# dachinzo/ringpop-node

Measured on AMD Instinct MI355X. Metric: ring lookups/s + member-updates merged/s; SWIM round time @100k members, higher is better.
Workload: dtype u32; 1 GPU; C2: 10000-server HashRing x 100 replica points, batched lookupN(n=3) of 36-byte keys, 2^26 keys per step; servers=10000, replica_points=100, total_keys=164550934528, parallelism=keys sharded, ring replicated

## Files before the change

### ringpop-node_amd/csrc/rp_ring.hip

```cpp
#include <algorithm>
#include <chrono>
#include <cstdio>
#include <cstdlib>
#include <cstring>
#include <memory>
#include <mutex>
#include <string>
#include <unordered_map>
#include <vector>

#include "../../include/ringpop_amd.h"
#include "rp_farmhash.h"
#include "rp_philox.h"
#include "rp_hashlong.h"
#include "rp_names.h"
#include "rp_prims.h"

namespace rp {

constexpr uint32_t NIL = 0xFFFFFFFFu;

static bool getenv_flag(const char* name) {
    const char* v = getenv(name);
    return v && *v && *v != '0';
// ... 926 lines not shown
        auto defer = [&](uint32_t kk) {
            const uint32_t sp = atomicAdd(&nslow_tile, 1u);
            if (sp < kSlowPerTile) slow_list[t * kSlowPerTile + sp] = kk;
        };
        constexpr int KH = KPL / LH;
        static_assert(KPL % LH == 0, "whole halves");
#ifdef RP_LK_PROF
        uint64_t t3 = 0;
#endif
#pragma unroll
        for (int hh = 0; hh < LH; hh++) {
        if (hh) __builtin_amdgcn_sched_barrier(0);
        u32x2 rec[KH];
#pragma unroll
        for (int kq = 0; kq < KH; kq++) rec[kq] = lk.index_rec(h[hh * KH + kq]);
        uint32_t lo[KH], bc[KH], ws[KH];
        u32x4 win[KH];
#pragma unroll
        for (int kq = 0; kq < KH; kq++) win[kq] = lk.window(h[hh * KH + kq], rec[kq], lo[kq], bc[kq], ws[kq]);
#ifdef RP_LK_PROF
        if (hh == 0) {
            LK_T(t3h, lo[KH - 1]);
            t3 = t3h;
        }
#endif
#pragma unroll
        for (int kq = 0; kq < KH; kq++) {
            const int k = hh * KH + kq;
            lk.resolve(win[kq], h[k], lo[kq], bc[kq], ws[kq], (uint32_t)(tid + k * kLkThreads), nag, ag[wv], so, cnt_tile,
                       defer);
        }
        }
        LK_T(t4, nag);
        __builtin_amdgcn_fence(__ATOMIC_SEQ_CST, "wavefront");
        for (uint32_t j = lane; j < (nag < AG ? nag : AG); j += 64)
            lk.finish2(lk.load16(ag[wv][0][j]), ag[wv][1][j], ag[wv][2][j], so, cnt_tile, defer);
        LK_T(t5a, nag);
        __syncthreads();
        LK_T(t5, tid);
        if (tid == 0) slow_cnt[t] = nslow_tile;
        u32x4* d4 = reinterpret_cast<u32x4*>(out + base * NEED);
        const u32x4* s4 = reinterpret_cast<const u32x4*>(so);
#pragma unroll
        for (int k = tid; k < TK * NEED / 4; k += kLkThreads) __builtin_nontemporal_store(s4[k], d4 + k);
        __syncthreads();
#ifdef RP_LK_PROF
        LK_T(t6, tid);
        pa[1] += t2 - t0;
        pa[2] += t3 - t2;
        pa[3] += t4 - t3;
        pa[4] += t5a - t4;
        pa[5] += t6 - t5;
        ntl += 1;
        (void)t5;
#endif
    }
#ifdef RP_LK_PROF
    if (lane == 0) {
        for (int i = 0; i < 6; i++) atomicAdd(&g_lk_prof[i], (unsigned long long)pa[i]);
        atomicAdd(&g_lk_prof[6], (unsigned long long)ntl);
    }
#endif
    if constexpr (FUSE) {
        constexpr uint32_t TPP = kLkThreads / kSlowPerTile;
        const uint64_t nt = ntiles > blockIdx.x ? (ntiles - blockIdx.x + gridDim.x - 1) / gridDim.x : 0;
        for (uint64_t i0 = 0; i0 < nt; i0 += TPP) {
            const uint64_t i = i0 + (uint32_t)tid / kSlowPerTile;
            const uint32_t q = (uint32_t)tid % kSlowPerTile;
            if (i < nt) {
                const uint64_t t = blockIdx.x + i * gridDim.x;
                const uint32_t c = slow_cnt[t];
                if (c <= kSlowPerTile) {
                    if (q < c) lookupn_redo(keys, fv, np, (uint32_t)NEED, out, counts, t * TK + slow_list[t * kSlowPerTile + q]);
                } else {
                    for (uint32_t k = q; k < (uint32_t)TK; k += kSlowPerTile) lookupn_redo(keys, fv, np, (uint32_t)NEED, out, counts, t * TK + k);
                }
            }
        }
    }
}

#ifdef RP_LK_PROF
__device__ unsigned long long g_sk_prof[10];
#endif
constexpr int kSortDefault = 256;

template <int THREADS, int NEED>
__global__ __launch_bounds__(THREADS) __attribute__((amdgpu_waves_per_eu(4))) void k_lookupn_sorted(
    const uint8_t* __restrict__ keys, uint64_t ntiles, CompactView cv, uint32_t* __restrict__ out,
    uint8_t* __restrict__ counts, uint32_t* __restrict__ slow_list, uint32_t* __restrict__ slow_cnt) {
    constexpr int LEN = 36, W4 = LEN / 4, KPL = 8, HS = 4;
    constexpr int TK = THREADS * KPL;
    constexpr int NW = THREADS / 64;
    constexpr int SUB = TK / 2048;
    constexpr int SK = TK * W4 / HS, SO = TK * NEED;
    constexpr int BINS = THREADS;
    constexpr int BSH = 32 - (BINS == 256 ? 8 : BINS == 512 ? 9 : 10);
    constexpr int CW = BINS / 2;
    constexpr int WPL = CW / 64;
    static_assert(THREADS == 256 || THREADS == 512 || THREADS == 1024, "whole 2,048-key logical tiles, 13-bit slots, 16-bit bin counters");
    static_assert(2 * TK <= SO && SK <= SO, "the ordered pairs and the key slice fit under the rows");
    __shared__ __attribute__((aligned(16))) uint32_t lds[SO];
    __shared__ uint32_t ag[NW][3][kLkAG];
    __shared__ uint32_t bins[CW];
    __shared__ uint32_t nslow_sub[SUB];
    uint32_t* const sk = lds;
    uint32_t* const so = lds;
    u32x2* const pairs = reinterpret_cast<u32x2*>(lds);
    const int tid = threadIdx.x, lane = tid & 63, wv = tid >> 6;
    const LkStages<NEED, 13> lk(cv);
#ifdef RP_LK_PROF
    uint64_t pa[6] = {0, 0, 0, 0, 0, 0}, ntl = 0;
#endif
    if (tid < CW) bins[tid] = 0;
    if (tid < SUB) nslow_sub[tid] = 0;
    for (uint64_t t = blockIdx.x; t < ntiles; t += gridDim.x) {
        const uint64_t base = t * TK;
        uint32_t h[KPL], kk[KPL];
        LK_T(t0, tid);
        lk_key_stage<64, KPL, HS, true>(keys + (base + (uint64_t)wv * 512) * LEN, sk + wv * (SK / NW), lane, h, [] {}, [] {});
        LK_T(t1, h[KPL - 1]);
        uint32_t rank[KPL];
#pragma unroll
        for (int k = 0; k < KPL; k++) {
            const uint32_t b = h[k] >> BSH, sh = (b & 1u) * 16u;
            rank[k] = (atomicAdd(&bins[b >> 1], 1u << sh) >> sh) & 0xFFFFu;
        }
        __syncthreads();
        if (wv == 0) {
            uint32_t c[WPL], sum = 0;
#pragma unroll
            for (int i = 0; i < WPL; i++) {
                c[i] = bins[lane * WPL + i];
                sum += (c[i] & 0xFFFFu) + (c[i] >> 16);
            }
            uint32_t x = sum;
#pragma unroll
            for (int o = 1; o < 64; o <<= 1) {
                const uint32_t y = __shfl_up(x, o, 64);
                if (lane >= o) x += y;
            }
            uint32_t run = x - sum;
#pragma unroll
            for (int i = 0; i < WPL; i++) {
                const uint32_t a = run, b = run + (c[i] & 0xFFFFu);
                run = b + (c[i] >> 16);
                bins[lane * WPL + i] = a | (b << 16);
            }
        }
        __syncthreads();
#pragma unroll
        for (int k = 0; k < KPL; k++) {
            const uint32_t b = h[k] >> BSH, sh = (b & 1u) * 16u;
            const uint32_t slot = ((bins[b >> 1] >> sh) & 0xFFFFu) + rank[k];
            pairs[slot] = u32x2{h[k], (uint32_t)(wv * 512 + lane + 64 * k)};
        }
        __syncthreads();
#pragma unroll
        for (int k = 0; k < KPL; k++) {
            const u32x2 p = pairs[tid + k * THREADS];
            h[k] = p.x;
            kk[k] = p.y;
        }
        if (tid < CW) bins[tid] = 0;
        if (tid < SUB) nslow_sub[tid] = 0;
        LK_T(t2, kk[KPL - 1]);
        __syncthreads();
        uint32_t nag = 0;
        uint8_t* const cnt_tile = counts ? counts + base : nullptr;
        auto defer = [&](uint32_t k) {
            const uint32_t s = k >> 11;
            const uint32_t sp = atomicAdd(&nslow_sub[s], 1u);
            if (sp < kSlowPerTile) slow_list[(t * SUB + s) * kSlowPerTile + sp] = k & 2047u;
        };
        u32x2 rec[KPL];
#pragma unroll
        for (int k = 0; k < KPL; k++) rec[k] = lk.index_rec(h[k]);
        uint32_t lo[KPL], bc[KPL], ws[KPL];
        u32x4 win[KPL];
#pragma unroll
        for (int k = 0; k < KPL; k++) win[k] = lk.window(h[k], rec[k], lo[k], bc[k], ws[k]);
        LK_T(t3, lo[KPL - 1]);
#pragma unroll
        for (int k = 0; k < KPL; k++) lk.resolve(win[k], h[k], lo[k], bc[k], ws[k], kk[k], nag, ag[wv], so, cnt_tile, defer);
        LK_T(t4, nag);
        __builtin_amdgcn_fence(__ATOMIC_SEQ_CST, "wavefront");
        for (uint32_t j = lane; j < (nag < kLkAG ? nag : kLkAG); j += 64)
            lk.finish2(lk.load16(ag[wv][0][j]), ag[wv][1][j], ag[wv][2][j], so, cnt_tile, defer);
        LK_T(t5a, nag);
        __syncthreads();
        LK_T(t5, tid);
        if (tid < SUB) slow_cnt[t * SUB + tid] = nslow_sub[tid];
        u32x4* d4 = reinterpret_cast<u32x4*>(out + base * NEED);
        const u32x4* s4 = reinterpret_cast<const u32x4*>(so);
#pragma unroll
        for (int k = tid; k < TK * NEED / 4; k += THREADS) __builtin_nontemporal_store(s4[k], d4 + k);
        __syncthreads();
#ifdef RP_LK_PROF
        LK_T(t6, tid);
        pa[0] += t1 - t0;
        pa[1] += t2 - t1;
        pa[2] += t3 - t2;
        pa[3] += t4 - t3;
        pa[4] += t5a - t4;
        pa[5] += t6 - t5;
        ntl += 1;
#endif
    }
#ifdef RP_LK_PROF
    if (lane == 0) {
        for (int i = 0; i < 6; i++) atomicAdd(&g_sk_prof[i], (unsigned long long)pa[i]);
        atomicAdd(&g_sk_prof[6], (unsigned long long)ntl);
    }
#endif
}

constexpr int kWsSlots = 2;
constexpr uint32_t kWsSpin = 1u << 22;
typedef uint32_t u32x3v __attribute__((ext_vector_type(3)));

template <int NP, int NC, int ABL = 0>
__global__ __launch_bounds__((NP + NC) * 64) __attribute__((amdgpu_waves_per_eu(4))) void k_lookupn_ws(const uint8_t* __restrict__ keys, uint64_t nwt,
                                                               CompactView cv, uint32_t* __restrict__ out,
                                                               uint32_t out_bytes, uint8_t* __restrict__ counts,
                                                               uint32_t* __restrict__ slow_list,
                                                               uint32_t* __restrict__ slow_cnt,
                                                               uint32_t* __restrict__ err) {
    constexpr int NEED = 3, KPL = 8, LEN = 36, W4 = LEN / 4;
    constexpr int TK = 64 * KPL;
    constexpr int V4 = TK * W4 / 4;
    constexpr int PER = V4 / 64;
    constexpr uint32_t SPAN = 5 - NEED;
    constexpr uint32_t AG = 64;
    static_assert(V4 % 64 == 0, "wave-tile shape");
    __shared__ __attribute__((aligned(16))) uint32_t stg[NP][V4 * 4];
    __shared__ uint32_t ring[NC][kWsSlots][TK];
    __shared__ uint32_t ag[NC][3][AG];
    __shared__ uint32_t prod[NC], cons[NC], nsl[NC];
    const int tid = threadIdx.x, lane = tid & 63, wv = tid >> 6;
    if (tid < NC) {
        prod[tid] = 0;
        cons[tid] = 0;
    }
    __syncthreads();
    const uint64_t nwg = (nwt + NC - 1) / NC;
    auto wait_ge = [&](uint32_t* p, uint32_t target) {
        for (uint32_t n = 0;; n++) {
            const uint32_t v = __builtin_amdgcn_readfirstlane(__hip_atomic_load(p, __ATOMIC_RELAXED, __HIP_MEMORY_SCOPE_WORKGROUP));
            if (v >= target) break;
            if (n == kWsSpin) {
                if (lane == 0) atomicOr(err, 1u);
                break;
            }
            __builtin_amdgcn_s_sleep(1);
            asm volatile("" ::: "memory");
        }
        asm volatile("" ::: "memory");
    };
    if (wv < NP) {
        const int cnt = (NC - wv + NP - 1) / NP;
        auto item_wt = [&](uint32_t j) -> uint64_t {
            const uint64_t T = blockIdx.x + (uint64_t)(j / cnt) * gridDim.x;
            const uint64_t wt = T * NC + wv + (j % cnt) * NP;
            return T < nwg && wt < nwt ? wt : ~0ull;
        };
        u32x4 pre[PER];
        auto issue = [&](uint64_t wt) {
            const u32x4* s4 = reinterpret_cast<const u32x4*>(keys + wt * (uint64_t)(TK * LEN));
#pragma unroll
            for (int q = 0; q < PER; q++) pre[q] = __builtin_nontemporal_load(s4 + lane + 64 * q);
        };
        uint64_t wt = item_wt(0);
        if (ABL != 1 && wt != ~0ull) issue(wt);
        for (uint32_t j = 0; wt != ~0ull; j++) {
            const uint64_t wn = item_wt(j + 1);
            uint32_t h[KPL];
            if constexpr (ABL == 1) {
#pragma unroll
                for (int k = 0; k < KPL; k++) h[k] = (uint32_t)(wt * TK + lane + 64 * k) * 0x9E3779B1u;
            } else {
                u32x4* st4 = reinterpret_cast<u32x4*>(stg[wv]);
#pragma unroll
                for (int q = 0; q < PER; q++) st4[lane + 64 * q] = pre[q];
                __builtin_amdgcn_wave_barrier();
                if (wn != ~0ull) issue(wn);
#pragma unroll
                for (int k = 0; k < KPL; k++) {
                    uint32_t w[W4];
#pragma unroll
                    for (int x = 0; x < W4; x++) w[x] = stg[wv][(lane + 64 * k) * W4 + x];
                    h[k] = fh::hash32_words<LEN>(w);
                }
            }
            __builtin_amdgcn_wave_barrier();
            const int c = wv + (int)(j % cnt) * NP;
            const uint32_t i = j / cnt;
            wait_ge(&cons[c], i + 1 > (uint32_t)kWsSlots ? i + 1 - kWsSlots : 0u);
// ... 1036 lines not shown
        const uint32_t p = pos[i];
        for (uint32_t q = lane; q < L; q += 64) buf[p + q] = names[b + q];
        if (lane == 0) buf[p + L] = ';';
    }
}

__global__ void k_hash_batch(const uint8_t* __restrict__ bytes, const uint64_t* __restrict__ off, uint64_t n,
                             uint32_t* __restrict__ out) {
    const uint64_t gstride = (uint64_t)gridDim.x * blockDim.x;
    for (uint64_t k = (uint64_t)blockIdx.x * blockDim.x + threadIdx.x; k < n; k += gstride)
        out[k] = fh::hash32(fh::PtrSrc{bytes + off[k]}, (uint32_t)(off[k + 1] - off[k]));
}

__global__ void k_gen_uuid(uint32_t seed, uint64_t k0, uint64_t n, uint32_t* __restrict__ out) {
    const uint64_t gstride = (uint64_t)gridDim.x * blockDim.x;
    for (uint64_t k = (uint64_t)blockIdx.x * blockDim.x + threadIdx.x; k < n; k += gstride) {
        uint32_t w[9];
        uuid_key_words(seed, k0 + k, w);
#pragma unroll
        for (int j = 0; j < 9; j++) out[k * 9 + j] = w[j];
    }
}

}


struct LoadScratch {
    DevBuf<uint32_t> rows;
    DevBuf<unsigned long long> out;
    StreamOrder order;
    void use_on(hipStream_t st) { order.use_on(st); }
};

struct RangeScratch {
    DevBuf<uint32_t> val, mi, mj;
    DevBuf<uint32_t> tot;
    DevBuf<uint8_t> flg;
    DevBuf<uint32_t> io;
    StreamOrder order;
    void use_on(hipStream_t st) { order.use_on(st); }
};

struct HandoffScratch {
    DevBuf<uint32_t> key, dst, src, perm;
    DevBuf<uint8_t> slot;
    DevBuf<uint32_t> rank;
    DevBuf<uint32_t> io;
    StreamOrder order;
    void use_on(hipStream_t st) { order.use_on(st); }
};

struct RouteScratch {
    DevBuf<unsigned long long> plane;
    DevBuf<unsigned long long> meta;
    DevBuf<uint8_t> tr;
    DevBuf<unsigned long long> scan;
    DevBuf<uint8_t> io8;
    DevBuf<uint32_t> io32;
    DevBuf<unsigned long long> io64;
    StreamOrder order;
    void use_on(hipStream_t st) { order.use_on(st); }
};

struct LookupKnobs {
    bool wide;
    bool layout_packed;
    bool nowindow;
    bool ablate_set;
    int ablate;
    bool wpred;
    bool hint;
    bool lds;
    uint64_t lds_grid;
    bool lds_stg;
    int lds_abl;
    bool ws;
    int ws_np, ws_nc;
    uint64_t ws_grid;
    int ws_abl;
    bool kpl_set;
    int kpl;
    int sort_t;
    uint64_t grid;
    bool lean_set;
    bool lean;
    bool half_set;
    int half;
    bool fusefix;
    bool stg_set;
    int stg;
    bool lh_set;
    uint64_t lh;
    uint64_t stghs;
    bool debug;
    bool prof_print;
};
static LookupKnobs lookup_knobs() {
    const auto num = [](const char* v) { return v ? atoi(v) : 0; };
    const auto is0 = [](const char* v) { return v && !strcmp(v, "0"); };
    const char *lay = getenv("RP_RING_LAYOUT"), *abl = getenv("RP_LOOKUP_ABLATE"), *lds = getenv("RP_LOOKUP_LDS"),
               *ws = getenv("RP_LOOKUP_WS"), *kpl = getenv("RP_LOOKUP_KPL"), *sort = getenv("RP_LOOKUP_SORT"),
               *lean = getenv("RP_LOOKUP_LEAN"), *half = getenv("RP_LOOKUP_HALF"), *stg = getenv("RP_LOOKUP_STG");
    LookupKnobs k;
    k.wide = getenv_flag("RP_RING_WIDE");
    k.layout_packed = lay && !strcmp(lay, "packed");
    k.nowindow = getenv_flag("RP_RING_NOWINDOW");
    k.ablate_set = abl != nullptr;
    k.ablate = num(abl);
    k.wpred = !is0(getenv("RP_LOOKUP_WPRED"));
    k.hint = !is0(getenv("RP_LOOKUP_HINT"));
    k.lds = lds ? !strcmp(lds, "1") : kLdsDefault;
    k.lds_grid = env_pos("RP_LOOKUP_LDS_GRID", 0);
    k.lds_stg = (int)env_pos("RP_LOOKUP_LDS_STG", 0) == 1;
    k.lds_abl = num(getenv("RP_LOOKUP_LDS_ABL"));
    k.ws = ws && !is0(ws);
    k.ws_np = 1, k.ws_nc = 3;
    if (k.ws && strchr(ws, ':') && sscanf(ws, "%d:%d", &k.ws_np, &k.ws_nc) != 2) k.ws_np = 0;
    k.ws_grid = env_pos("RP_LOOKUP_WS_GRID", 0);
    k.ws_abl = num(getenv("RP_LOOKUP_WS_ABL"));
    k.kpl_set = kpl != nullptr;
    k.kpl = num(kpl);
    k.sort_t = sort ? atoi(sort) : kSortDefault;
    k.grid = env_pos("RP_LOOKUP_GRID", 0);
    k.lean_set = lean != nullptr;
    k.lean = !is0(lean);
    k.half_set = half != nullptr;
    k.half = num(half);
    k.fusefix = getenv_flag("RP_LOOKUP_FUSEFIX");
    k.stg_set = stg != nullptr;
    k.stg = num(stg);
    k.lh_set = getenv("RP_LOOKUP_LH") != nullptr;
    k.lh = env_pos("RP_LOOKUP_LH", 0);
    k.stghs = env_pos("RP_LOOKUP_STGHS", 8);
    k.debug = getenv_flag("RP_LOOKUP_DEBUG");
    k.prof_print = getenv_flag("RP_LK_PROF_PRINT");
    return k;
}

struct Ring {
    int device = 0;
    hipStream_t st = nullptr;
    uint32_t R = 100;
    NameTable nt;
    std::vector<uint8_t> in_ring;
    std::vector<uint64_t> stamp;
    uint64_t next_stamp = 1;
    uint32_t server_count = 0;
    bool has_checksum = false;
    uint32_t checksum = 0;
    DevBuf<uint32_t> tok, own, tok2, own2, bstart;
    uint32_t M = 0;
    uint32_t bbits = 8;
    DevBuf<uint32_t> ent, pbstart;
    DevBuf<uint32_t> slow, nslow;
    bool packed = false;
    uint32_t pbits = 16;
    DevBuf<uint8_t> cent;
    DevBuf<uint32_t> cidx;
    DevBuf<uint32_t> cidxh;
    bool chint = false;
    bool chint_pending = false;
    bool compact = false;
    uint32_t ccb = 0, cob = 0, cfsh = 0;
    DevBuf<uint8_t> lent;
    DevBuf<uint4> lidx;
    bool lds = false, lds_pending = false;
    uint32_t lng = 0, llg = 0, lfb = 0;
    DevBuf<uint8_t> d_inring;
    DevBuf<uint8_t> ck_buf;
    DevBuf<uint32_t> ck_out;
    DevBuf<uint32_t> ntok, nown, flag, pos, ids_dev, tmpk;
    DevBuf<uint64_t> tmp64;
    DevBuf<uint32_t> scalar;
    DevBuf<uint32_t> io_a, io_b;
    DevBuf<uint8_t> io_keys, io_cnt;
    uint32_t* pin_out = nullptr;
    uint8_t* pin_cnt = nullptr;
    uint32_t* pin_out_dev = nullptr;
    uint8_t* pin_cnt_dev = nullptr;
    DevBuf<uint64_t> io_off;
    SvcLines* svc = nullptr;
    SvcLines* svc_dev = nullptr;
    hipStream_t svc_st = nullptr;
    uint32_t svc_idle_ms = 0, svc_seq = 0;
    std::atomic<bool> svc_live{false};
    std::recursive_mutex svc_mu;
    bool svc_v2 = true;
    DevBuf<uint4> svc_dt;
    uint32_t svc_dtb = 0;
    bool svc_dt_valid = false;
    uint64_t svc_prof[9] = {0, 0, 0, 0, 0, 0, 0, 0, 0};
    DevBuf<uint32_t> grp_own, grp_key, grp_first, grp_dk, grp_dv, grp_rank;
    Scratch ws;
    LoadScratch load_ws;
    RangeScratch range_ws;
    HandoffScratch handoff_ws;
    RouteScratch route_ws;
    uint32_t inring_n = 0;

    RingView view() const {
        return RingView{tok.p, own.p, bstart.p, M, 32u - bbits};
    }
    PackedView pview() const { return PackedView{ent.p, pbstart.p, M, pbits}; }
    CompactView cview(const LookupKnobs& k) const {
        return CompactView{cent.p, cidx.p, M, ccb, cob, cfsh, cfsh == 0, (uint32_t)k.ablate,
                           (uint32_t)(3ull * ((uint64_t)M + kEnt3Pad + 6) + 16), (uint32_t)(8ull << (ccb - 3)),
                           k.wpred ? 1u : 0u, chint && k.hint ? cidxh.p : nullptr};
    }
};

struct Replicas {
    int np;
    uint32_t W;
};
static Replicas replicas(int32_t nrep, uint32_t servers) {
    return {(int)std::min<int64_t>(nrep, servers), nrep > 1 ? (uint32_t)nrep : 1u};
}

static uint32_t ring_intern(Ring& r, const char* s, uint32_t n) {
    const uint32_t id = r.nt.intern(s, n);
    if (id >= r.in_ring.size()) {
        r.in_ring.resize(id + 1, 0);
        r.stamp.resize(id + 1, 0);
    }
    return id;
}

static uint32_t choose_bbits(uint32_t M) {
    uint32_t b = 8;
    while (b < 22 && (1ull << (b + 2)) < M) b++;
    return b;
}

static void ring_build_compact(Ring& r) {
    r.compact = false;
    if (r.M < 64) return;
    uint32_t ob = 1;
// ... 301 lines not shown
        hipLaunchKernelGGL(kern, dim3(g), dim3(kLdsThreads), 0, b.st, b.keys, nwt, lv, b.out, b.counts, r.slow.p,
                           r.nslow.p);
    };
    if (b.need == 3 && k.lds_abl) {
        switch (k.lds_abl) {
            case 1: tiles(k_lookupn_lds<KPL, 3, 0, 1>); break;
            case 2: tiles(k_lookupn_lds<KPL, 3, 0, 2>); break;
            case 3: tiles(k_lookupn_lds<KPL, 3, 0, 3>); break;
            case 4: tiles(k_lookupn_lds<KPL, 3, 0, 4>); break;
            default: tiles(k_lookupn_lds<KPL, 3, 0, 7>); break;
        }
    } else {
        with_need(b.need, [&](auto need) {
            constexpr int N = decltype(need)::value;
            if (k.lds_stg)
                tiles(k_lookupn_lds<KPL, N, 1, 0>);
            else
                tiles(k_lookupn_lds<KPL, N, 0, 0>);
        });
    }
    RP_HIP(hipGetLastError());
    lookupn_tiles_end(r, k, b, nwt, TK, nwt * TK, true, 0,
                      [&](auto done, auto tot, auto over, const uint32_t*) {
                          fprintf(stderr, "[rp] lds lookupN: %llu keys, %llu deferred, %llu overflowed tiles (ng %u fb %u ob %u)\n",
                                  done, tot, over, r.lng, r.lfb, r.cob);
                      });
    return true;
}

static bool lookupn_ws(Ring& r, const LookupKnobs& k, const Batch36& b, const CompactView& cv) {
    const uint64_t n = b.n;
    if (!k.ws || b.need != 3 || k.kpl_set || cv.ablate != 0 || n < 512ull * 4 || n * 12ull >= (1ull << 31))
        return false;
    const int wnp = k.ws_np, wnc = k.ws_nc;
    constexpr uint64_t TK = 512;
    const uint64_t nwt = n / TK;
    r.slow.reserve(nwt * kSlowPerTile + 1);
    r.nslow.reserve(nwt + 2);
    uint32_t* err = r.nslow.p + nwt + 1;
    RP_HIP(hipMemsetAsync(err, 0, 4, b.st));
    const uint64_t nwg = (nwt + (uint64_t)wnc - 1) / (uint64_t)(wnc > 0 ? wnc : 1);
    const uint64_t lds_wg = (uint64_t)wnp * 18432 + (uint64_t)wnc * (kWsSlots * 2048 + 780);
    const uint64_t per_cu = wnp + wnc > 0 ? std::max<uint64_t>(1, std::min<uint64_t>(16 / (uint64_t)(wnp + wnc), 163840 / lds_wg)) : 1;
    const unsigned g = (unsigned)std::min<uint64_t>(nwg, k.ws_grid ? k.ws_grid : (uint64_t)cu_count(r.device) * per_cu);
    using Kernel = decltype(&k_lookupn_ws<1, 3>);
    static const struct { int np, nc, abl; Kernel kern; } shapes[] = {
        {1, 3, 0, k_lookupn_ws<1, 3>},      {2, 6, 0, k_lookupn_ws<2, 6>},      {1, 7, 0, k_lookupn_ws<1, 7>},
        {4, 12, 1, k_lookupn_ws<4, 12, 1>}, {4, 12, 2, k_lookupn_ws<4, 12, 2>}, {4, 12, 0, k_lookupn_ws<4, 12>},
        {2, 2, 0, k_lookupn_ws<2, 2>},      {1, 15, 0, k_lookupn_ws<1, 15>},    {2, 14, 0, k_lookupn_ws<2, 14>}};
    Kernel kern = nullptr;
    for (const auto& s : shapes)
        if (!kern && s.np == wnp && s.nc == wnc && (s.abl == 0 || s.abl == k.ws_abl)) kern = s.kern;
    RP_REQUIRE(kern, "RP_LOOKUP_WS: one of 1:3, 2:6, 1:7, 4:12, 2:2, 1:15, 2:14");
    hipLaunchKernelGGL(kern, dim3(g), dim3((wnp + wnc) * 64), 0, b.st, b.keys, nwt, cv, b.out, (uint32_t)(n * 12ull), b.counts,
                       r.slow.p, r.nslow.p, err);
    RP_HIP(hipGetLastError());
    lookupn_tiles_end(r, k, b, nwt, TK, nwt * TK, true, 2,
                      [&](auto done, auto tot, auto over, const uint32_t* c) {
                          fprintf(stderr, "[rp] ws lookupN %d:%d: %llu keys, %llu deferred, %llu overflowed wave-tiles, err %u\n", wnp,
                                  wnc, done, tot, over, c[nwt + 1]);
                      });
    return true;
}

static void lookupn_compact(Ring& r, const LookupKnobs& k, const Batch36& b, const CompactView& cv) {
    const uint64_t n = b.n;
    const int need = b.need, np = b.np;
    const hipStream_t st = b.st;
    int kpl = k.kpl_set ? k.kpl : (need == 3 ? 8 : 4);
    if (kpl != 1 && kpl != 2 && !((kpl == 3 || kpl == 8) && need == 3)) kpl = 4;
    int sort_t = k.sort_t;
    RP_REQUIRE(sort_t == 0 || sort_t == 256 || sort_t == 512 || sort_t == 1024, "RP_LOOKUP_SORT: one of 0, 256, 512, 1024");
    if (need != 3 || !cv.idxh || cv.ablate != 0 || n < 8ull * (uint64_t)sort_t || k.kpl_set || k.half_set ||
        k.lean_set || k.stg_set || k.lh_set || k.fusefix)
        sort_t = 0;
    const uint64_t stiles = sort_t ? n / (8ull * (uint64_t)sort_t) : 0;
    const uint64_t s0 = stiles * 8ull * (uint64_t)sort_t;
    const uint64_t t0 = s0 / 2048;
    if (!sort_t && n < (uint64_t)kLkThreads * kpl) kpl = 4;
    const uint64_t TK = (uint64_t)kLkThreads * kpl;
    const uint64_t ntiles = (n - s0) / TK, done = s0 + ntiles * TK;
    r.slow.reserve((t0 + ntiles) * kSlowPerTile + 1);
    r.nslow.reserve(t0 + ntiles + 1);
    if (stiles) {
        const unsigned sg = grid_for(stiles, 1, (unsigned)(k.grid ? k.grid : sort_t == 256 ? 4096u : sort_t == 512 ? 8192u : 1024u));
        const auto sorted = [&](auto kern) {
            hipLaunchKernelGGL(kern, dim3(sg), dim3(sort_t), 0, st, b.keys, stiles, cv, b.out, b.counts, r.slow.p, r.nslow.p);
        };
        if (sort_t == 256)
            sorted(k_lookupn_sorted<256, 3>);
        else if (sort_t == 512)
            sorted(k_lookupn_sorted<512, 3>);
        else
            sorted(k_lookupn_sorted<1024, 3>);
        RP_HIP(hipGetLastError());
    }
    const bool lean = k.lean;
    const unsigned g = grid_for(ntiles, 1, (unsigned)(k.grid ? k.grid : lean ? 4096u : 2048u));
    const int half = k.half_set ? k.half : (kpl == 8 ? 4 : 0);
    const CompactFixView fv{r.tok.p, r.own.p, r.cidx.p, r.view(), r.M, r.ccb};
    const bool fuse = k.fusefix && lean && half == 4 && kpl == 8 && need == 3 && cv.ablate != 3;
    const bool stg1 = k.stg == 1 && lean && half == 4 && kpl == 8 && need == 3 && !fuse;
    const bool stg2 = lean && kpl == 8 && need == 3 && !fuse && k.stg == 2;
    const int lh = (lean && (half == 4 || stg2) && kpl == 8 && need == 3 && !fuse)
                       ? (int)(k.lh ? k.lh : (stg2 ? 2u : 1u)) : 1;
    const int stghs = (int)k.stghs;
    const auto tiles = [&](auto kern, auto... fix) {
        hipLaunchKernelGGL(kern, dim3(g), dim3(kLkThreads), 0, st, b.keys + s0 * 36, ntiles, cv, b.out + s0 * b.W,
                           b.counts ? b.counts + s0 : nullptr, r.slow.p + t0 * kSlowPerTile, r.nslow.p + t0, fix...);
    };
    const auto run = [&](auto keys_per_lane, auto owners) {
        constexpr int KPL = decltype(keys_per_lane)::value, NEED = decltype(owners)::value;
        if (!lean) return tiles(k_lookupn_compact<KPL, NEED>);
        if constexpr (KPL == 8 && NEED == 3) {
            if (stg2 && stghs == 8 && lh == 1) return tiles(k_lookupn_lean<8, 3, 8, false, 2, 1>, fv, np);
            if (stg2 && stghs == 8) return tiles(k_lookupn_lean<8, 3, 8, false, 2, 2>, fv, np);
            if (stg2) return tiles(k_lookupn_lean<8, 3, 4, false, 2, 2>, fv, np);
            if (stg1 && lh == 2) return tiles(k_lookupn_lean<8, 3, 4, false, 1, 2>, fv, np);
            if (lh == 2) return tiles(k_lookupn_lean<8, 3, 4, false, 0, 2>, fv, np);
            if (stg1) return tiles(k_lookupn_lean<8, 3, 4, false, 1>, fv, np);
        }
        if (half == 4 && KPL % 4 == 0 && fuse) return tiles(k_lookupn_lean<KPL, NEED, (KPL % 4 == 0 ? 4 : 1), true>, fv, np);
        if (half == 4 && KPL % 4 == 0) return tiles(k_lookupn_lean<KPL, NEED, (KPL % 4 == 0 ? 4 : 1)>, fv, np);
        if (half == 2 && KPL % 2 == 0) return tiles(k_lookupn_lean<KPL, NEED, (KPL % 2 == 0 ? 2 : 1)>, fv, np);
        return tiles(k_lookupn_lean<KPL, NEED>, fv, np);
    };
    if (ntiles == 0) {
    } else if (kpl == 1) {
        with_need(need, [&](auto owners) { run(Int<1>{}, owners); });
    } else if (kpl == 2) {
        with_need(need, [&](auto owners) { run(Int<2>{}, owners); });
    } else if (kpl == 8 && need == 3) {
        run(Int<8>{}, Int<3>{});
    } else if (kpl == 3 && need == 3) {
        run(Int<3>{}, Int<3>{});
    } else {
        with_need(need, [&](auto owners) { run(Int<4>{}, owners); });
    }
#ifdef RP_LK_PROF
    if (k.prof_print) {
        unsigned long long v[10];
        RP_HIP(hipStreamSynchronize(st));
        RP_HIP(hipMemcpyFromSymbol(v, HIP_SYMBOL(g_lk_prof), sizeof v));
        const double nw = (double)(v[6] ? v[6] : 1);
        fprintf(stderr,
                "[rp] lean phase cycles per wave-tile (%llu): keys-arrive %.0f hash-all %.0f idx %.0f win1+loop %.0f "
                "finish2 %.0f barrier+store %.0f\n",
                v[6], v[0] / nw, v[1] / nw, v[2] / nw, v[3] / nw, v[4] / nw, v[5] / nw);
        memset(v, 0, sizeof v);
        RP_HIP(hipMemcpyToSymbol(HIP_SYMBOL(g_lk_prof), v, sizeof v));
        if (stiles) {
            RP_HIP(hipMemcpyFromSymbol(v, HIP_SYMBOL(g_sk_prof), sizeof v));
            const double sw = (double)(v[6] ? v[6] : 1);
            fprintf(stderr,
                    "[rp] sorted<%d> phase cycles per wave-tile (%llu): keys+hash %.0f sort+deal %.0f idx+win-issue %.0f "
                    "win1+loop %.0f finish2 %.0f barrier+store %.0f\n",
                    sort_t, v[6], v[0] / sw, v[1] / sw, v[2] / sw, v[3] / sw, v[4] / sw, v[5] / sw);
            memset(v, 0, sizeof v);
            RP_HIP(hipMemcpyToSymbol(HIP_SYMBOL(g_sk_prof), v, sizeof v));
        }
    }
#endif
    lookupn_tiles_end(r, k, b, t0 + ntiles, TK, done, cv.ablate != 3 && !fuse, 0,
                      [&](auto keys_done, auto tot, auto over, const uint32_t*) {
                          fprintf(stderr, "[rp] compact lookupN: %llu keys, %llu deferred, %llu overflowed tiles (cb %u ob %u fsh %u sort %d)\n",
                                  keys_done, tot, over, r.ccb, r.cob, r.cfsh, sort_t);
                      });
}

static bool lookupn_probe(Ring& r, const LookupKnobs& k, const Batch36& b) {
    if (b.W > 4 || b.need > 4 || k.nowindow) return false;
    RP_REQUIRE(b.n < (1ull << 32), "lookupn: at most 2^32-1 keys per call");
    r.slow.reserve(b.n + 1);
    r.nslow.reserve(1);
    RP_HIP(hipMemsetAsync(r.nslow.p, 0, sizeof(uint32_t), b.st));
    const int kpl = k.kpl_set ? k.kpl : kDefaultKPL;
    const PackedView pv = r.pview();
    const auto probe = [&](auto keys_per_lane, auto mode) {
        constexpr int KPL = decltype(keys_per_lane)::value, MODE = decltype(mode)::value;
        hipLaunchKernelGGL((k_lookupn_probe<36, KPL, MODE>), dim3(grid_for(b.n, kLkThreads * KPL, 256 * 8)),
                           dim3(kLkThreads), 0, b.st, b.keys, b.n, pv, b.np, b.W, b.out, b.counts, r.slow.p, r.nslow.p);
        hipLaunchKernelGGL((k_lookupn_fix<36, MODE>), dim3(256), dim3(256), 0, b.st, b.keys, pv, b.np, b.W, b.out,
                           b.counts, r.slow.p, r.nslow.p);
    };
    if (k.ablate == 1)
        probe(Int<2>{}, Int<1>{});
    else if (k.ablate == 2)
        probe(Int<2>{}, Int<2>{});
    else if (kpl == 1)
        probe(Int<1>{}, Int<0>{});
    else if (kpl == 4)
        probe(Int<4>{}, Int<0>{});
    else if (kpl == 8)
        probe(Int<8>{}, Int<0>{});
    else
        probe(Int<2>{}, Int<0>{});
    RP_HIP(hipGetLastError());
    return true;
}

static void launch_lookupn(Ring& r, const uint8_t* keys, const uint64_t* off, uint32_t stride,
                           const uint32_t* hashes, uint64_t n, int np, uint32_t W, uint32_t* out, uint8_t* counts,
                           hipStream_t st) {
    if (n == 0) return;
    if (st != r.st) RP_HIP(hipStreamSynchronize(r.st));
    const LookupKnobs k = lookup_knobs();
    const bool fixed36 = DevKeys{keys, off, stride, hashes}.fixed36();
    const int need = np <= 0 ? 1 : np;
    const bool use_packed = r.packed && !k.wide;
    const bool use_compact = r.compact && !k.layout_packed && !k.wide;
    const bool aligned16 = ((reinterpret_cast<uintptr_t>(keys) & 15) == 0) && ((reinterpret_cast<uintptr_t>(out) & 15) == 0);
    const Batch36 b{keys, n, np, need, W, out, counts, st};
    const bool tiled = use_compact && fixed36 && aligned16 && (uint32_t)need == W && W <= 4;
    if (tiled && lookupn_lds(r, k, b)) return;
    if (tiled && n >= (uint64_t)kLkThreads * 4) {
        RP_REQUIRE(n < (1ull << 32), "lookupn: at most 2^32-1 keys per call");
        if (r.chint_pending && need == 3) ring_build_hint(r);
        const CompactView cv = r.cview(k);
        if (!lookupn_ws(r, k, b, cv)) lookupn_compact(r, k, b, cv);
        return;
    }
    if (use_packed && fixed36 && lookupn_probe(r, k, b)) return;
    if (use_packed)
        launch_lookupn_view(r.pview(), keys, off, stride, hashes, n, np, W, out, counts, st, k.ablate);
    else
        launch_lookupn_view(r.view(), keys, off, stride, hashes, n, np, W, out, counts, st, k.ablate);
}


__global__ void k_grp_first(const uint32_t* __restrict__ own, uint64_t n, uint32_t* __restrict__ first) {
    const uint64_t gstride = (uint64_t)gridDim.x * blockDim.x;
    for (uint64_t i = (uint64_t)blockIdx.x * blockDim.x + threadIdx.x; i < n; i += gstride) {
        const uint32_t s = own[i];
        if ((uint32_t)i < first[s]) atomicMin(first + s, (uint32_t)i);
    }
}

__global__ void k_grp_dest_keys(const uint32_t* __restrict__ first, uint32_t S, uint32_t n,
                                uint32_t* __restrict__ dk, uint32_t* __restrict__ dv) {
    const uint32_t gstride = gridDim.x * blockDim.x;
    for (uint32_t s = blockIdx.x * blockDim.x + threadIdx.x; s < S; s += gstride) {
        const uint32_t f = first[s];
        dk[s] = f < n ? f : n;
        dv[s] = s;
    }
}

__global__ void k_grp_rank(const uint32_t* __restrict__ dk, const uint32_t* __restrict__ dv, uint32_t S, uint32_t n,
                           uint32_t* __restrict__ rank, uint32_t* __restrict__ dests, uint32_t* __restrict__ ndest) {
// ... 2426 lines not shown
```

Before: 79.85 billion lookupN(3)/s.

## Add persistent ticket-scheduled sorted lookupN kernel with occupancy-sized grid

After: 82.49 billion lookupN(3)/s (median of 6 runs). 3.3% higher.

```diff
diff --git a/ringpop-node_amd/csrc/rp_ring.hip b/ringpop-node_amd/csrc/rp_ring.hip
--- a/ringpop-node_amd/csrc/rp_ring.hip
+++ b/ringpop-node_amd/csrc/rp_ring.hip
@@ -1032,8 +1032,37 @@
 
 #ifdef RP_LK_PROF
 __device__ unsigned long long g_sk_prof[10];
+#define RP_LK_TL
+#endif
+#ifdef RP_LK_TL
+constexpr uint32_t kTlMaxWg = 16384, kTlMaxTiles = 32768;
+__device__ unsigned long long g_tl_wg[2 * kTlMaxWg];
+__device__ uint32_t g_tl_hw[2 * kTlMaxWg];
+__device__ unsigned long long g_tl_tile[kTlMaxTiles];
+__device__ uint32_t g_tl_tile_wg[kTlMaxTiles];
+#define RP_TL_BEGIN()                                                                  \
+    if (threadIdx.x == 0 && blockIdx.x < kTlMaxWg) {                                   \
+        g_tl_wg[2 * blockIdx.x] = __builtin_amdgcn_s_memrealtime();                    \
+        g_tl_hw[2 * blockIdx.x] = __builtin_amdgcn_s_getreg(4 | (31 << 11));        \
+        g_tl_hw[2 * blockIdx.x + 1] = __builtin_amdgcn_s_getreg(20 | (31 << 11));  \
+    }
+#define RP_TL_TILE(t)                                      \
+    if (threadIdx.x == 0 && (t) < kTlMaxTiles) {           \
+        g_tl_tile[t] = __builtin_amdgcn_s_memrealtime();   \
+        g_tl_tile_wg[t] = blockIdx.x;                      \
+    }
+#define RP_TL_END() \
+    if (threadIdx.x == 0 && blockIdx.x < kTlMaxWg) g_tl_wg[2 * blockIdx.x + 1] = __builtin_amdgcn_s_memrealtime()
+#else
+#define RP_TL_BEGIN()
+#define RP_TL_TILE(t)
+#define RP_TL_END()
 #endif
 constexpr int kSortDefault = 256;
+constexpr bool kTicketDefault = true;
+constexpr int kStaggerDefault = 0;
+constexpr uint64_t kSortedTileUs = 25;
+constexpr uint32_t kStaggerSlots = 4;
 
 template <int THREADS, int NEED>
 __global__ __launch_bounds__(THREADS) __attribute__((amdgpu_waves_per_eu(4))) void k_lookupn_sorted(
@@ -1062,6 +1091,7 @@
 #ifdef RP_LK_PROF
     uint64_t pa[6] = {0, 0, 0, 0, 0, 0}, ntl = 0;
 #endif
+    RP_TL_BEGIN();
     if (tid < CW) bins[tid] = 0;
     if (tid < SUB) nslow_sub[tid] = 0;
     for (uint64_t t = blockIdx.x; t < ntiles; t += gridDim.x) {
@@ -1156,6 +1186,7 @@
         pa[5] += t6 - t5;
         ntl += 1;
 #endif
+        RP_TL_TILE(t);
     }
 #ifdef RP_LK_PROF
     if (lane == 0) {
@@ -1163,6 +1194,158 @@
         atomicAdd(&g_sk_prof[6], (unsigned long long)ntl);
     }
 #endif
+    RP_TL_END();
+}
+
+template <int THREADS, int NEED>
+__global__ __launch_bounds__(THREADS) __attribute__((amdgpu_waves_per_eu(4))) void k_lookupn_sorted_ticket(
+    const uint8_t* __restrict__ keys, uint64_t ntiles, CompactView cv, uint32_t* __restrict__ out,
+    uint8_t* __restrict__ counts, uint32_t* __restrict__ slow_list, uint32_t* __restrict__ slow_cnt,
+    uint32_t* __restrict__ tick, uint32_t stagger, uint32_t slot_div) {
+    constexpr int LEN = 36, W4 = LEN / 4, KPL = 8, HS = 4;
+    constexpr int TK = THREADS * KPL;
+    constexpr int NW = THREADS / 64;
+    constexpr int SUB = TK / 2048;
+    constexpr int SK = TK * W4 / HS, SO = TK * NEED;
+    constexpr int BINS = THREADS;
+    constexpr int BSH = 32 - (BINS == 256 ? 8 : BINS == 512 ? 9 : 10);
+    constexpr int CW = BINS / 2;
+    constexpr int WPL = CW / 64;
+    static_assert(THREADS == 256 || THREADS == 512 || THREADS == 1024, "whole 2,048-key logical tiles, 13-bit slots, 16-bit bin counters");
+    static_assert(2 * TK <= SO && SK <= SO, "the ordered pairs and the key slice fit under the rows");
+    __shared__ __attribute__((aligned(16))) uint32_t lds[SO];
+    __shared__ uint32_t ag[NW][3][kLkAG];
+    __shared__ uint32_t bins[CW];
+    __shared__ uint32_t nslow_sub[SUB];
+    __shared__ uint32_t next_tile;
+    uint32_t* const sk = lds;
+    uint32_t* const so = lds;
+    u32x2* const pairs = reinterpret_cast<u32x2*>(lds);
+    const int tid = threadIdx.x, lane = tid & 63, wv = tid >> 6;
+    const LkStages<NEED, 13> lk(cv);
+#ifdef RP_LK_PROF
+    uint64_t pa[6] = {0, 0, 0, 0, 0, 0}, ntl = 0;
+#endif
+    RP_TL_BEGIN();
+    if (tid < CW) bins[tid] = 0;
+    if (tid < SUB) nslow_sub[tid] = 0;
+    const uint32_t naps = ((blockIdx.x / slot_div) % kStaggerSlots) * stagger;
+    for (uint32_t i = 0; i < naps; i++) __builtin_amdgcn_s_sleep(16);
+    uint64_t nxt = 0;
+    uint32_t zero;
+    asm("v_mov_b32 %0, 0" : "=v"(zero));
+    for (uint64_t t = blockIdx.x; t < ntiles; t = nxt) {
+        const uint64_t base = t * TK;
+        uint32_t h[KPL], kk[KPL];
+        uint32_t drawn = 0;
+        if (tid == 0) drawn = __hip_atomic_fetch_add(tick + zero, 1u, __ATOMIC_RELAXED, __HIP_MEMORY_SCOPE_AGENT);
+        LK_T(t0, tid);
+        lk_key_stage<64, KPL, HS, true>(keys + (base + (uint64_t)wv * 512) * LEN, sk + wv * (SK / NW), lane, h, [] {}, [] {});
+        LK_T(t1, h[KPL - 1]);
+        uint32_t rank[KPL];
+#pragma unroll
+        for (int k = 0; k < KPL; k++) {
+            const uint32_t b = h[k] >> BSH, sh = (b & 1u) * 16u;
+            rank[k] = (atomicAdd(&bins[b >> 1], 1u << sh) >> sh) & 0xFFFFu;
+        }
+        if (tid == 0) next_tile = drawn;
+        __syncthreads();
+        if (wv == 0) {
+            uint32_t c[WPL], sum = 0;
+#pragma unroll
+            for (int i = 0; i < WPL; i++) {
+                c[i] = bins[lane * WPL + i];
+                sum += (c[i] & 0xFFFFu) + (c[i] >> 16);
+            }
+            uint32_t x = sum;
+#pragma unroll
+            for (int o = 1; o < 64; o <<= 1) {
+                const uint32_t y = __shfl_up(x, o, 64);
+                if (lane >= o) x += y;
+            }
+            uint32_t run = x - sum;
+#pragma unroll
+            for (int i = 0; i < WPL; i++) {
+                const uint32_t a = run, b = run + (c[i] & 0xFFFFu);
+                run = b + (c[i] >> 16);
+                bins[lane * WPL + i] = a | (b << 16);
+            }
+        }
+        __syncthreads();
+#pragma unroll
+        for (int k = 0; k < KPL; k++) {
+            const uint32_t b = h[k] >> BSH, sh = (b & 1u) * 16u;
+            const uint32_t slot = ((bins[b >> 1] >> sh) & 0xFFFFu) + rank[k];
+            pairs[slot] = u32x2{h[k], (uint32_t)(wv * 512 + lane + 64 * k)};
+        }
+        __syncthreads();
+#pragma unroll
+        for (int k = 0; k < KPL; k++) {
+            const u32x2 p = pairs[tid + k * THREADS];
+            h[k] = p.x;
+            kk[k] = p.y;
+        }
+        if (tid < CW) bins[tid] = 0;
+        if (tid < SUB) nslow_sub[tid] = 0;
+        LK_T(t2, kk[KPL - 1]);
+        __syncthreads();
+        uint32_t nag = 0;
+        uint8_t* const cnt_tile = counts ? counts + base : nullptr;
+        auto defer = [&](uint32_t k) {
+            const uint32_t s = k >> 11;
+            const uint32_t sp = atomicAdd(&nslow_sub[s], 1u);
+            if (sp < kSlowPerTile) slow_list[(t * SUB + s) * kSlowPerTile + sp] = k & 2047u;
+        };
+        u32x2 rec[KPL];
+#pragma unroll
+        for (int k = 0; k < KPL; k++) rec[k] = lk.index_rec(h[k]);
+        uint32_t lo[KPL], bc[KPL], ws[KPL];
+        u32x4 win[KPL];
+#pragma unroll
+        for (int k = 0; k < KPL; k++) win[k] = lk.window(h[k], rec[k], lo[k], bc[k], ws[k]);
+        LK_T(t3, lo[KPL - 1]);
+#pragma unroll
+        for (int k = 0; k < KPL; k++) lk.resolve(win[k], h[k], lo[k], bc[k], ws[k], kk[k], nag, ag[wv], so, cnt_tile, defer);
+        LK_T(t4, nag);
+        __builtin_amdgcn_fence(__ATOMIC_SEQ_CST, "wavefront");
+        for (uint32_t j = lane; j < (nag < kLkAG ? nag : kLkAG); j += 64)
+            lk.finish2(lk.load16(ag[wv][0][j]), ag[wv][1][j], ag[wv][2][j], so, cnt_tile, defer);
+        LK_T(t5a, nag);
+        __syncthreads();
+        LK_T(t5, tid);
+        nxt = (uint64_t)gridDim.x + next_tile;
+        if (tid < SUB) slow_cnt[t * SUB + tid] = nslow_sub[tid];
+        u32x4* d4 = reinterpret_cast<u32x4*>(out + base * NEED);
+        const u32x4* s4 = reinterpret_cast<const u32x4*>(so);
+#pragma unroll
+        for (int k = tid; k < TK * NEED / 4; k += THREADS) __builtin_nontemporal_store(s4[k], d4 + k);
+        __syncthreads();
+#ifdef RP_LK_PROF
+        LK_T(t6, tid);
+        pa[0] += t1 - t0;
+        pa[1] += t2 - t1;
+        pa[2] += t3 - t2;
+        pa[3] += t4 - t3;
+        pa[4] += t5a - t4;
+        pa[5] += t6 - t5;
+        ntl += 1;
+#endif
+        RP_TL_TILE(t);
+    }
+#ifdef RP_LK_PROF
+    if (lane == 0) {
+        for (int i = 0; i < 6; i++) atomicAdd(&g_sk_prof[i], (unsigned long long)pa[i]);
+        atomicAdd(&g_sk_prof[6], (unsigned long long)ntl);
+    }
+#endif
+    RP_TL_END();
+    if (tid == 0) {
+        const uint32_t left = __hip_atomic_fetch_add(tick + 1, 1u, __ATOMIC_RELAXED, __HIP_MEMORY_SCOPE_AGENT);
+        if (left + 1u == gridDim.x) {
+            __hip_atomic_store(tick, 0u, __ATOMIC_RELAXED, __HIP_MEMORY_SCOPE_AGENT);
+            __hip_atomic_store(tick + 1, 0u, __ATOMIC_RELAXED, __HIP_MEMORY_SCOPE_AGENT);
+        }
+    }
 }
 
 constexpr int kWsSlots = 2;
@@ -2365,6 +2548,10 @@
     int kpl;
     int sort_t;
     uint64_t grid;
+    int ticket;
+    int stagger;
+    uint64_t ticket_grid;
+    const char* tl_dump;
     bool lean_set;
     bool lean;
     bool half_set;
@@ -2383,7 +2570,8 @@
     const auto is0 = [](const char* v) { return v && !strcmp(v, "0"); };
     const char *lay = getenv("RP_RING_LAYOUT"), *abl = getenv("RP_LOOKUP_ABLATE"), *lds = getenv("RP_LOOKUP_LDS"),
                *ws = getenv("RP_LOOKUP_WS"), *kpl = getenv("RP_LOOKUP_KPL"), *sort = getenv("RP_LOOKUP_SORT"),
-               *lean = getenv("RP_LOOKUP_LEAN"), *half = getenv("RP_LOOKUP_HALF"), *stg = getenv("RP_LOOKUP_STG");
+               *lean = getenv("RP_LOOKUP_LEAN"), *half = getenv("RP_LOOKUP_HALF"), *stg = getenv("RP_LOOKUP_STG"),
+               *tick = getenv("RP_LOOKUP_TICKET"), *stag = getenv("RP_LOOKUP_STAGGER");
     LookupKnobs k;
     k.wide = getenv_flag("RP_RING_WIDE");
     k.layout_packed = lay && !strcmp(lay, "packed");
@@ -2405,6 +2593,10 @@
     k.kpl = num(kpl);
     k.sort_t = sort ? atoi(sort) : kSortDefault;
     k.grid = env_pos("RP_LOOKUP_GRID", 0);
+    k.ticket = tick ? (is0(tick) ? 0 : 1) : -1;
+    k.stagger = stag ? std::min(std::max(atoi(stag), 0), 64) : -1;
+    k.ticket_grid = env_pos("RP_LOOKUP_TICKET_GRID", 0);
+    k.tl_dump = getenv("RP_LK_TL_DUMP");
     k.lean_set = lean != nullptr;
     k.lean = !is0(lean);
     k.half_set = half != nullptr;
@@ -2436,6 +2628,8 @@
     uint32_t bbits = 8;
     DevBuf<uint32_t> ent, pbstart;
     DevBuf<uint32_t> slow, nslow;
+    DevBuf<uint32_t> tick;
+    int ticket_per_cu = 0;
     bool packed = false;
     uint32_t pbits = 16;
     DevBuf<uint8_t> cent;
@@ -2903,8 +3097,31 @@
     const uint64_t ntiles = (n - s0) / TK, done = s0 + ntiles * TK;
     r.slow.reserve((t0 + ntiles) * kSlowPerTile + 1);
     r.nslow.reserve(t0 + ntiles + 1);
-    if (stiles) {
-        const unsigned sg = grid_for(stiles, 1, (unsigned)(k.grid ? k.grid : sort_t == 256 ? 4096u : sort_t == 512 ? 8192u : 1024u));
+    const bool ticket = stiles && sort_t == 256 && !k.grid && (k.ticket < 0 ? kTicketDefault : k.ticket == 1);
+    unsigned sg = 0;
+    int stag16 = 0;
+    if (ticket) {
+        if (!r.tick.p) {
+            r.tick.reserve(2);
+            RP_HIP(hipMemsetAsync(r.tick.p, 0, 2 * sizeof(uint32_t), st));
+            RP_HIP(hipStreamSynchronize(st));
+        }
+        if (!r.ticket_per_cu) {
+            int nbl = 0;
+            RP_HIP(hipOccupancyMaxActiveBlocksPerMultiprocessor(&nbl, reinterpret_cast<const void*>(k_lookupn_sorted_ticket<256, 3>), 256, 0));
+            r.ticket_per_cu = std::max(nbl, 1);
+        }
+        const uint64_t cus = (uint64_t)cu_count(r.device);
+        sg = (unsigned)(k.ticket_grid ? std::min<uint64_t>(k.ticket_grid, 1u << 20) : std::min<uint64_t>(cus * (uint64_t)r.ticket_per_cu, stiles));
+        stag16 = k.stagger < 0 ? kStaggerDefault : k.stagger;
+        int khz = 0;
+        if (stag16) (void)hipDeviceGetAttribute(&khz, hipDeviceAttributeClockRate, r.device);
+        const uint32_t naps = (uint32_t)((uint64_t)stag16 * kSortedTileUs * (uint64_t)(khz > 0 ? khz / 1000 : 2400) / (16u * 1024u));
+        hipLaunchKernelGGL((k_lookupn_sorted_ticket<256, 3>), dim3(sg), dim3(256), 0, st, b.keys, stiles, cv, b.out, b.counts,
+                           r.slow.p, r.nslow.p, r.tick.p, naps, (uint32_t)cus);
+        RP_HIP(hipGetLastError());
+    } else if (stiles) {
+        sg = grid_for(stiles, 1, (unsigned)(k.grid ? k.grid : sort_t == 256 ? 4096u : sort_t == 512 ? 8192u : 1024u));
         const auto sorted = [&](auto kern) {
             hipLaunchKernelGGL(kern, dim3(sg), dim3(sort_t), 0, st, b.keys, stiles, cv, b.out, b.counts, r.slow.p, r.nslow.p);
         };
@@ -2982,10 +3199,31 @@
         }
     }
 #endif
+#ifdef RP_LK_TL
+    if (k.tl_dump && stiles) {
+        const uint32_t nwg = std::min<uint32_t>(sg, kTlMaxWg), nt = (uint32_t)std::min<uint64_t>(stiles, kTlMaxTiles);
+        std::vector<unsigned long long> wg(2 * kTlMaxWg), te(kTlMaxTiles);
+        std::vector<uint32_t> hw(2 * kTlMaxWg), tw(kTlMaxTiles);
+        RP_HIP(hipStreamSynchronize(st));
+        RP_HIP(hipMemcpyFromSymbol(wg.data(), HIP_SYMBOL(g_tl_wg), 8 * wg.size()));
+        RP_HIP(hipMemcpyFromSymbol(hw.data(), HIP_SYMBOL(g_tl_hw), 4 * hw.size()));
+        RP_HIP(hipMemcpyFromSymbol(te.data(), HIP_SYMBOL(g_tl_tile), 8 * te.size()));
+        RP_HIP(hipMemcpyFromSymbol(tw.data(), HIP_SYMBOL(g_tl_tile_wg), 4 * tw.size()));
+        if (FILE* f = fopen(k.tl_dump, "w")) {
+            fprintf(f, "# sort %d ticket %d grid %u stagger %d tiles %llu\n", sort_t, ticket ? 1 : 0, sg, stag16,
+                    (unsigned long long)stiles);
+            for (uint32_t i = 0; i < nwg; i++)
+                fprintf(f, "W %u %u %u %llu %llu\n", i, hw[2 * i], hw[2 * i + 1], wg[2 * i], wg[2 * i + 1]);
+            for (uint32_t i = 0; i < nt; i++) fprintf(f, "T %u %u %llu\n", i, tw[i], te[i]);
+            fclose(f);
+        }
+    }
+#endif
     lookupn_tiles_end(r, k, b, t0 + ntiles, TK, done, cv.ablate != 3 && !fuse, 0,
                       [&](auto keys_done, auto tot, auto over, const uint32_t*) {
-                          fprintf(stderr, "[rp] compact lookupN: %llu keys, %llu deferred, %llu overflowed tiles (cb %u ob %u fsh %u sort %d)\n",
-                                  keys_done, tot, over, r.ccb, r.cob, r.cfsh, sort_t);
+                          fprintf(stderr, "[rp] compact lookupN: %llu keys, %llu deferred, %llu overflowed tiles (cb %u ob %u fsh %u sort %d) "
+                                          "ticket %d grid %u stagger %d\n",
+                                  keys_done, tot, over, r.ccb, r.cob, r.cfsh, sort_t, ticket ? 1 : 0, sg, stag16);
                       });
 }
 
```
